# yangdongchao/Text-to-sound-Synthesis

Hardware: NVIDIA H100
Metric: clips/sec (10s audio, 100 diffusion steps) (higher is better)
Workload: dtype f16x3

## Files before the change

### include/diffsound_b200.h

```cpp
#ifndef DIFFSOUND_B200_H
#define DIFFSOUND_B200_H

#include <stdint.h>

#ifdef __cplusplus
extern "C" {
#endif

#define DSB_VERSION 100

#define DSB_DTYPE_TF32 0
#define DSB_DTYPE_BF16 1
#define DSB_DTYPE_F16 2

#define DSB_GEMM_GELU2 1
#define DSB_GEMM_ROUND_TF32 2
#define DSB_GEMM_OUT_BF16 4
#define DSB_GEMM_LRELU 8
#define DSB_GEMM_TANH 16
#define DSB_GEMM_OUT_F16 256
#define DSB_GEMM_RES_BEFORE_ACT 128
#define DSB_GEMM_DUAL_LRELU 4096
#define DSB_GEMM_NO_STORE 16384
#define DSB_GEMM_RELU 32768
// ... 33 lines not shown
  int b_mn_major;
  int use_tap_wcol;
  int tap_wcol[32];
  long long w_cols;
  long long split_off;
  long long dual_off;
  int out_col_group;
  int out_col_group_stride;
  const void* A2;
  long long a2_rows, a2_cols, lda2, a2_batch_stride;
  int tap_a2[32];
  float* amax_out;
  int resident_w;
  int schedule;
} dsb_gemm_desc;
int dsb_gemm_ex(const dsb_gemm_desc* desc, void* stream);

int dsb_gemm_f32(const float* A, const float* W, const float* bias, const float* residual, float* out, int M, int N, int K,
                 long long lda, long long ldw, long long ldo, long long ld_res, int flags, void* stream);

int dsb_round_tf32(const float* in, float* out, long long n, void* stream);
int dsb_f32_to_bf16(const float* in, void* out_bf16, long long n, void* stream);
int dsb_f32_to_f16(const float* in, void* out_f16, long long n, void* stream);
int dsb_split_f16(const float* in, long long ld_in, void* out_f16, long long ld_out, long long lo_off, long long rows, int C, float scale,
                  void* stream);
int dsb_split_tf32(const float* in, long long ld_in, float* out, long long ld_out, long long rows, int C, int Cp, int w_format, void* stream);

int dsb_embed_tokens(const int64_t* ids, const float* emb, const float* height_emb, const float* width_emb, float* out, int B, int L,
                     int D, int H, int W, int num_embed, int* err_flag, void* stream);

int dsb_layernorm(const float* x, void* out, const float* gamma, const float* beta, int rows, int D, float eps, int flags, void* stream);

int dsb_ada_layernorm(const float* x, void* out, const float* table, const int64_t* t, int B, int L, int D, int T, float eps, int flags,
                      void* stream);

int dsb_l2_normalize_rows(float* x, long long rows, int D, void* stream);

int dsb_silu(const float* in, float* out, long long n, void* stream);

int dsb_attention(const float* q, long long ldq, const float* k, long long ldk, const float* v, long long ldv, float* o, long long ldo,
                  int B, int H, int Lq, int Lk, float scale, int flags, void* stream);

#define DSB_ATTN_CAUSAL 1024
int dsb_attention_f16(const void* q, long long ldq, const void* k, long long ldk, const void* v, long long ldv, void* o, long long ldo,
                      int B, int H, int Lq, int Lk, float scale, int flags, void* stream);

int dsb_attention_tc(const void* q, long long ldq, const void* k, long long ldk, const void* v, long long ldv, void* o, long long ldo,
                     int B, int H, int Lq, int Lk, float scale, void* stream);
int dsb_attention_tc2(const void* q, long long ldq, const void* k, long long ldk, const void* v, long long ldv, void* o, long long ldo,
                      int B, int H, int Lq, int Lk, float scale, void* stream);
int dsb_attention_tc_split(const void* q, long long ldq, long long q_lo_off, const void* k, long long ldk, long long k_lo_off, const void* v,
                           long long ldv, long long v_lo_off, void* o, long long ldo, long long o_lo_off, int B, int H, int Lq, int Lk,
                           float scale, void* stream);


#define DSB_STAGE_INPUT_LOGPROB 1
#define DSB_STAGE_SKIP_POSTERIOR 2
#define DSB_STAGE_SKIP_SAMPLE 4
int dsb_posterior_sample(const float* logits, const int64_t* x_t, const int64_t* t, const int64_t* t_post, const float* uniform,
                         const float* sched, int64_t* x_next, float* log_prob_out, int B, int K, int L, int T, int trunc_mode,
                         float trunc_r, int trunc_k, int stage_flags, void* stream);

int dsb_posterior_sample_loop(const float* logits, int64_t* x, int64_t* t, int64_t* t_post, const float* sched, unsigned long long* ctrl,
                              const int64_t* t_sched, const int64_t* t_post_sched, int B, int K, int L, int T, int trunc_mode, float trunc_r,
                              int trunc_k, void* stream);
int dsb_posterior_sample_wide(const float* logits, const int64_t* x_t, const int64_t* t, const int64_t* t_post, const float* uniform,
                              const float* sched, int64_t* x_next, float* log_prob_out, int B, int K, int L, int T, int trunc_mode,
                              float trunc_r, int trunc_k, int stage_flags, void* stream);
int dsb_posterior_sample_wide_loop(const float* logits, int64_t* x, int64_t* t, int64_t* t_post, const float* sched, unsigned long long* ctrl,
                                   const int64_t* t_sched, const int64_t* t_post_sched, int B, int K, int L, int T, int trunc_mode, float trunc_r,
                                   int trunc_k, void* stream);
int dsb_aten_uniform(float* out, long long n, unsigned long long seed, unsigned long long offset, unsigned long long nthreads, void* stream);
int dsb_aten_exponential(float* out, long long n, unsigned long long seed, unsigned long long offset, unsigned long long nthreads, void* stream);

int dsb_ar_embed(const float* cond, const float* tok_emb, const float* pos_emb, const int64_t* ids, long long ids_ld, float* x,
                 const unsigned long long* ctrl, int B, int Tc, int V, int D, int* err_flag, void* stream);
int dsb_ar_attention(const float* qkv, long long ld_qkv, float* k_cache, float* v_cache, long long cache_ld, int max_pos, void* out, long long ld_out,
                     long long lo_off, const unsigned long long* ctrl, int B, int H, int head_dim, float scale, void* stream);
int dsb_gelu_erf_split(const float* in, long long ld_in, void* out, long long ld_out, long long lo_off, int rows, int C, void* stream);
int dsb_ar_sample(const float* logits, long long ld_logits, int64_t* ids, long long ids_ld, unsigned long long* ctrl, int B, int V, int Tc,
                  float temperature, int top_k, int do_sample, float* probs_out, float* logits_hist, long long hist_ld, int* err_flag, void* stream);

int dsb_codebook_gather_padded(const int64_t* ids, const float* codebook, float* out, int B, int H, int W, int E, int n_codes, int flags,
                               int* err_flag, void* stream);
int dsb_groupnorm_stats(const float* x, double* stats, int B, int P, int C, int groups, void* stream);
int dsb_groupnorm_apply(const float* x, const double* stats, const float* gamma, const float* beta, float* out, int B, int H, int W, int C,
                        int groups, float eps, int flags, int Lp, void* stream);
int dsb_upsample2x_padded(const float* in, float* out, int B, int H, int W, int C, int flags, void* stream);
int dsb_softmax_rows(float* x, long long rows, int n_valid, int ld, int flags, void* stream);
int dsb_space_to_depth_padded(const float* in, float* out, int B, int H, int W, int C, int flags, void* stream);
int dsb_row_argmin(const float* x, long long ld, long long rows, int n, int64_t* out, void* stream);
int dsb_tokens_add_to_padded(const float* tok, float* xpad, int B, int H, int W, int C, int Lp, void* stream);

int dsb_lrelu_pad(const float* in, float* out, int B, int T, int C, int pad, float slope, int reflect, int in_channel_major, int flags,
                  void* stream);
int dsb_mel_pack_f16(const float* mel, void* out_f16, int B, int Cm, int T, int pad, int Kp, void* stream);
int dsb_edge_pad_f16(void* state_f16, long long ld, long long batch_stride, int B, int T, int P, int d, int col0, int ncols, int reflect,
                     void* stream);
int dsb_conv_out_pair(const void* state, long long ld, long long batch_stride, int B, int T, int row0, int col0, int cs, int kt, const float* w,
                      const float* bias, float scale, float* out, void* stream);


int dsb_mel_stem(const float* x, const float* mean, const float* stdv, const float* w, const float* bias, float scale, void* out, int B, int F, int T,
                 int Cout, int Hp, int Wp, int y0, int x0, void* stream);
int dsb_pair_space_to_depth(const void* in, int Hpi, int Wpi, int y0, int x0, int H, int W, void* out, int Hpo, int Wpo, int oy0, int ox0, int B, int C,
                            void* stream);
// ... 43 lines not shown
```

### text-to-sound-synthesis_b200/_lib.py

```python
from __future__ import annotations

import ctypes as C
import os

_HERE = os.path.dirname(os.path.abspath(__file__))
LIB_PATH = os.path.join(_HERE, "libdiffsound_b200.so")

c_vp, c_i, c_ll, c_f = C.c_void_p, C.c_int, C.c_longlong, C.c_float


class GemmDesc(C.Structure):
    _fields_ = [
        ("A", c_vp), ("W", c_vp), ("bias", c_vp), ("residual", c_vp), ("out", c_vp),
        ("M", c_i), ("N", c_i), ("K", c_i), ("batch", c_i),
        ("a_rows", c_ll), ("lda", c_ll), ("ldw", c_ll), ("ldo", c_ll), ("ld_res", c_ll),
        ("a_batch_stride", c_ll), ("w_batch_stride", c_ll), ("out_batch_stride", c_ll), ("res_batch_stride", c_ll),
        ("dtype", c_i), ("flags", c_i), ("num_taps", c_i), ("tap_shift", c_i * 32), ("tap_acol", c_i * 32), ("a_cols", c_ll),
        ("geo_P", c_i), ("geo_Wp", c_i), ("geo_y0", c_i), ("geo_y1", c_i), ("geo_x0", c_i), ("geo_x1", c_i),
        ("alpha", c_f), ("block_n", c_i), ("max_ctas", c_i), ("cta_pair", c_i), ("a_mn_major", c_i), ("b_mn_major", c_i),
        ("use_tap_wcol", c_i), ("tap_wcol", c_i * 32), ("w_cols", c_ll), ("split_off", c_ll),
        ("dual_off", c_ll), ("out_col_group", c_i), ("out_col_group_stride", c_i), ("A2", c_vp),
        ("a2_rows", c_ll), ("a2_cols", c_ll), ("lda2", c_ll), ("a2_batch_stride", c_ll), ("tap_a2", c_i * 32), ("amax_out", c_vp), ("resident_w", c_i),
        ("schedule", c_i),
    ]


SIGNATURES = {
    "dsb_version": [],
    "dsb_device_info": [C.POINTER(c_i)] * 3,
    "dsb_gemm_ex": [C.POINTER(GemmDesc), c_vp],
    "dsb_gemm_f32": [c_vp] * 5 + [c_i] * 3 + [c_ll] * 4 + [c_i, c_vp],
    "dsb_round_tf32": [c_vp, c_vp, c_ll, c_vp],
    "dsb_f32_to_bf16": [c_vp, c_vp, c_ll, c_vp],
    "dsb_f32_to_f16": [c_vp, c_vp, c_ll, c_vp],
    "dsb_silu": [c_vp, c_vp, c_ll, c_vp],
    "dsb_split_f16": [c_vp, c_ll, c_vp, c_ll, c_ll, c_ll, c_i, c_f, c_vp],
    "dsb_attention_tc_split": [c_vp, c_ll, c_ll, c_vp, c_ll, c_ll, c_vp, c_ll, c_ll, c_vp, c_ll, c_ll, c_i, c_i, c_i, c_i, c_f, c_vp],
    "dsb_l2_normalize_rows": [c_vp, c_ll, c_i, c_vp],
    "dsb_split_tf32": [c_vp, c_ll, c_vp, c_ll, c_ll, c_i, c_i, c_i, c_vp],
    "dsb_embed_tokens": [c_vp] * 5 + [c_i] * 6 + [c_vp, c_vp],
    "dsb_layernorm": [c_vp] * 4 + [c_i, c_i, c_f, c_i, c_vp],
    "dsb_ada_layernorm": [c_vp] * 4 + [c_i] * 4 + [c_f, c_i, c_vp],
    "dsb_attention": [c_vp, c_ll, c_vp, c_ll, c_vp, c_ll, c_vp, c_ll, c_i, c_i, c_i, c_i, c_f, c_i, c_vp],
    "dsb_codebook_gather_padded": [c_vp] * 3 + [c_i] * 6 + [c_vp, c_vp],
    "dsb_groupnorm_stats": [c_vp, c_vp] + [c_i] * 4 + [c_vp],
    "dsb_groupnorm_apply": [c_vp] * 5 + [c_i] * 5 + [c_f, c_i, c_i, c_vp],
    "dsb_upsample2x_padded": [c_vp, c_vp] + [c_i] * 5 + [c_vp],
    "dsb_softmax_rows": [c_vp, c_ll, c_i, c_i, c_i, c_vp],
    "dsb_space_to_depth_padded": [c_vp, c_vp] + [c_i] * 5 + [c_vp],
    "dsb_row_argmin": [c_vp, c_ll, c_ll, c_i, c_vp, c_vp],
    "dsb_tokens_add_to_padded": [c_vp, c_vp] + [c_i] * 5 + [c_vp],
    "dsb_lrelu_pad": [c_vp, c_vp] + [c_i] * 4 + [c_f, c_i, c_i, c_i, c_vp],
    "dsb_mel_pack_f16": [c_vp, c_vp] + [c_i] * 5 + [c_vp],
    "dsb_edge_pad_f16": [c_vp, c_ll, c_ll] + [c_i] * 7 + [c_vp],
    "dsb_conv_out_pair": [c_vp, c_ll, c_ll] + [c_i] * 6 + [c_vp, c_vp, c_f, c_vp, c_vp],
    "dsb_attention_f16": [c_vp, c_ll, c_vp, c_ll, c_vp, c_ll, c_vp, c_ll, c_i, c_i, c_i, c_i, c_f, c_i, c_vp],
    "dsb_attention_tc2": [c_vp, c_ll, c_vp, c_ll, c_vp, c_ll, c_vp, c_ll, c_i, c_i, c_i, c_i, c_f, c_vp],
    "dsb_attention_tc": [c_vp, c_ll, c_vp, c_ll, c_vp, c_ll, c_vp, c_ll, c_i, c_i, c_i, c_i, c_f, c_vp],
    "dsb_posterior_sample": [c_vp] * 8 + [c_i] * 5 + [c_f, c_i, c_i, c_vp],
    "dsb_posterior_sample_loop": [c_vp] * 8 + [c_i] * 5 + [c_f, c_i, c_vp],
    "dsb_posterior_sample_wide": [c_vp] * 8 + [c_i] * 5 + [c_f, c_i, c_i, c_vp],
    "dsb_posterior_sample_wide_loop": [c_vp] * 8 + [c_i] * 5 + [c_f, c_i, c_vp],
    "dsb_aten_uniform": [c_vp, c_ll, C.c_ulonglong, C.c_ulonglong, C.c_ulonglong, c_vp],
    "dsb_aten_exponential": [c_vp, c_ll, C.c_ulonglong, C.c_ulonglong, C.c_ulonglong, c_vp],
    "dsb_ar_embed": [c_vp] * 4 + [c_ll, c_vp, c_vp] + [c_i] * 4 + [c_vp, c_vp],
    "dsb_ar_attention": [c_vp, c_ll, c_vp, c_vp, c_ll, c_i, c_vp, c_ll, c_ll, c_vp, c_i, c_i, c_i, c_f, c_vp],
    "dsb_gelu_erf_split": [c_vp, c_ll, c_vp, c_ll, c_ll, c_i, c_i, c_vp],
    "dsb_ar_sample": [c_vp, c_ll, c_vp, c_ll, c_vp, c_i, c_i, c_i, c_f, c_i, c_i, c_vp, c_vp, c_ll, c_vp, c_vp],
    "dsb_mel_stem": [c_vp] * 5 + [c_f, c_vp] + [c_i] * 8 + [c_vp],
    "dsb_pair_space_to_depth": [c_vp] + [c_i] * 6 + [c_vp] + [c_i] * 6 + [c_vp],
    "dsb_pair_maxpool3s2": [c_vp] + [c_i] * 6 + [c_vp, c_ll, c_ll] + [c_i] * 6 + [c_f, c_vp],
    "dsb_pair_avgpool3": [c_vp] + [c_i] * 6 + [c_vp, c_ll, c_ll, c_i, c_i, c_vp],
    "dsb_pair_channel_mean": [c_vp, c_ll, c_ll] + [c_i] * 8 + [c_f, c_vp, c_vp],
    "dsb_q_sample": [c_vp] * 5 + [c_i] * 4 + [c_vp],
    "dsb_train_loss": [c_vp] * 16 + [c_i] * 4 + [c_f, c_i, c_f, c_f, c_i, c_vp],
    "dsb_transpose": [c_vp, c_ll, c_ll, c_vp, c_ll, c_ll, c_i, c_i, c_i, c_i, c_vp],
    "dsb_heads_split": [c_vp, c_ll, c_vp, c_i, c_i, c_i, c_i, c_vp],
    "dsb_heads_merge": [c_vp, c_vp, c_ll, c_i, c_i, c_i, c_i, c_vp],
    "dsb_cast_scale": [c_vp, c_vp, c_ll, c_vp, c_i, c_vp],
    "dsb_colsum": [c_vp, c_ll, c_vp, c_ll, c_i, c_i, c_vp],
    "dsb_gelu2_fwd": [c_vp, c_vp, c_ll, c_i, c_vp],
    "dsb_gelu2_bwd": [c_vp, c_vp, c_vp, c_ll, c_i, c_vp],
    "dsb_silu_bwd": [c_vp, c_vp, c_vp, c_ll, c_vp],
    "dsb_gather_rows": [c_vp, c_vp, c_vp, c_i, c_i, c_vp],
    "dsb_scatter_add_rows": [c_vp, c_vp, c_vp, c_i, c_i, c_vp],
    "dsb_layernorm_bwd": [c_vp] * 6 + [c_ll, c_i, c_f, c_vp, c_i, c_vp],
    "dsb_ada_layernorm_bwd": [c_vp] * 6 + [c_i, c_i, c_i, c_f, c_vp, c_i, c_vp],
    "dsb_softmax_fwd": [c_vp, c_ll, c_vp, c_ll, c_ll, c_i, c_i, c_vp],
    "dsb_softmax_bwd": [c_vp, c_ll, c_vp, c_ll, c_vp, c_ll, c_ll, c_i, c_f, c_i, c_vp],
    "dsb_embed_bwd": [c_vp] * 5 + [c_i] * 6 + [c_vp],
# ... 28 lines not shown
```

### text-to-sound-synthesis_b200/csrc/wgmma.cuh

```cuda
#pragma once
#include "common.cuh"
#include "diffsound_b200.h"

namespace dsb {

template <int KIND, int TA, int TB>
__device__ __forceinline__ void wgmma_m64n128(float (&d)[64], uint64_t da, uint64_t db, uint32_t scale_d) {
  static_assert(KIND != DSB_DTYPE_TF32 || (TA == 0 && TB == 0), "tf32 wgmma takes K-major operands only");
  if constexpr (KIND == DSB_DTYPE_TF32) {
    asm volatile(
        "{\n\t.reg .pred p;\n\tsetp.ne.b32 p, %66, 0;\n\t"
        "wgmma.mma_async.sync.aligned.m64n128k8.f32.tf32.tf32 "
        "{%0, %1, %2, %3, %4, %5, %6, %7, %8, %9, %10, %11, %12, %13, %14, %15, %16, %17, %18, %19, %20, %21, %22, %23, %24, %25, %26, %27, %28, %29, %30, %31, %32, %33, %34, %35, %36, %37, %38, %39, %40, %41, %42, %43, %44, %45, %46, %47, %48, %49, %50, %51, %52, %53, %54, %55, %56, %57, %58, %59, %60, %61, %62, %63}, "
        "%64, %65, p, 1, 1;\n\t}"
        : "+f"(d[0]), "+f"(d[1]), "+f"(d[2]), "+f"(d[3]), "+f"(d[4]), "+f"(d[5]), "+f"(d[6]), "+f"(d[7]), "+f"(d[8]), "+f"(d[9]), "+f"(d[10]), "+f"(d[11]), "+f"(d[12]), "+f"(d[13]), "+f"(d[14]), "+f"(d[15]), "+f"(d[16]), "+f"(d[17]), "+f"(d[18]), "+f"(d[19]), "+f"(d[20]), "+f"(d[21]), "+f"(d[22]), "+f"(d[23]), "+f"(d[24]), "+f"(d[25]), "+f"(d[26]), "+f"(d[27]), "+f"(d[28]), "+f"(d[29]), "+f"(d[30]), "+f"(d[31]), "+f"(d[32]), "+f"(d[33]), "+f"(d[34]), "+f"(d[35]), "+f"(d[36]), "+f"(d[37]), "+f"(d[38]), "+f"(d[39]), "+f"(d[40]), "+f"(d[41]), "+f"(d[42]), "+f"(d[43]), "+f"(d[44]), "+f"(d[45]), "+f"(d[46]), "+f"(d[47]), "+f"(d[48]), "+f"(d[49]), "+f"(d[50]), "+f"(d[51]), "+f"(d[52]), "+f"(d[53]), "+f"(d[54]), "+f"(d[55]), "+f"(d[56]), "+f"(d[57]), "+f"(d[58]), "+f"(d[59]), "+f"(d[60]), "+f"(d[61]), "+f"(d[62]), "+f"(d[63])
        : "l"(da), "l"(db), "r"(scale_d));
  } else if constexpr (KIND == DSB_DTYPE_BF16) {
    asm volatile(
        "{\n\t.reg .pred p;\n\tsetp.ne.b32 p, %66, 0;\n\t"
        "wgmma.mma_async.sync.aligned.m64n128k16.f32.bf16.bf16 "
        "{%0, %1, %2, %3, %4, %5, %6, %7, %8, %9, %10, %11, %12, %13, %14, %15, %16, %17, %18, %19, %20, %21, %22, %23, %24, %25, %26, %27, %28, %29, %30, %31, %32, %33, %34, %35, %36, %37, %38, %39, %40, %41, %42, %43, %44, %45, %46, %47, %48, %49, %50, %51, %52, %53, %54, %55, %56, %57, %58, %59, %60, %61, %62, %63}, "
        "%64, %65, p, 1, 1, %67, %68;\n\t}"
        : "+f"(d[0]), "+f"(d[1]), "+f"(d[2]), "+f"(d[3]), "+f"(d[4]), "+f"(d[5]), "+f"(d[6]), "+f"(d[7]), "+f"(d[8]), "+f"(d[9]), "+f"(d[10]), "+f"(d[11]), "+f"(d[12]), "+f"(d[13]), "+f"(d[14]), "+f"(d[15]), "+f"(d[16]), "+f"(d[17]), "+f"(d[18]), "+f"(d[19]), "+f"(d[20]), "+f"(d[21]), "+f"(d[22]), "+f"(d[23]), "+f"(d[24]), "+f"(d[25]), "+f"(d[26]), "+f"(d[27]), "+f"(d[28]), "+f"(d[29]), "+f"(d[30]), "+f"(d[31]), "+f"(d[32]), "+f"(d[33]), "+f"(d[34]), "+f"(d[35]), "+f"(d[36]), "+f"(d[37]), "+f"(d[38]), "+f"(d[39]), "+f"(d[40]), "+f"(d[41]), "+f"(d[42]), "+f"(d[43]), "+f"(d[44]), "+f"(d[45]), "+f"(d[46]), "+f"(d[47]), "+f"(d[48]), "+f"(d[49]), "+f"(d[50]), "+f"(d[51]), "+f"(d[52]), "+f"(d[53]), "+f"(d[54]), "+f"(d[55]), "+f"(d[56]), "+f"(d[57]), "+f"(d[58]), "+f"(d[59]), "+f"(d[60]), "+f"(d[61]), "+f"(d[62]), "+f"(d[63])
        : "l"(da), "l"(db), "r"(scale_d), "n"(TA), "n"(TB));
  } else {
    asm volatile(
        "{\n\t.reg .pred p;\n\tsetp.ne.b32 p, %66, 0;\n\t"
        "wgmma.mma_async.sync.aligned.m64n128k16.f32.f16.f16 "
        "{%0, %1, %2, %3, %4, %5, %6, %7, %8, %9, %10, %11, %12, %13, %14, %15, %16, %17, %18, %19, %20, %21, %22, %23, %24, %25, %26, %27, %28, %29, %30, %31, %32, %33, %34, %35, %36, %37, %38, %39, %40, %41, %42, %43, %44, %45, %46, %47, %48, %49, %50, %51, %52, %53, %54, %55, %56, %57, %58, %59, %60, %61, %62, %63}, "
        "%64, %65, p, 1, 1, %67, %68;\n\t}"
        : "+f"(d[0]), "+f"(d[1]), "+f"(d[2]), "+f"(d[3]), "+f"(d[4]), "+f"(d[5]), "+f"(d[6]), "+f"(d[7]), "+f"(d[8]), "+f"(d[9]), "+f"(d[10]), "+f"(d[11]), "+f"(d[12]), "+f"(d[13]), "+f"(d[14]), "+f"(d[15]), "+f"(d[16]), "+f"(d[17]), "+f"(d[18]), "+f"(d[19]), "+f"(d[20]), "+f"(d[21]), "+f"(d[22]), "+f"(d[23]), "+f"(d[24]), "+f"(d[25]), "+f"(d[26]), "+f"(d[27]), "+f"(d[28]), "+f"(d[29]), "+f"(d[30]), "+f"(d[31]), "+f"(d[32]), "+f"(d[33]), "+f"(d[34]), "+f"(d[35]), "+f"(d[36]), "+f"(d[37]), "+f"(d[38]), "+f"(d[39]), "+f"(d[40]), "+f"(d[41]), "+f"(d[42]), "+f"(d[43]), "+f"(d[44]), "+f"(d[45]), "+f"(d[46]), "+f"(d[47]), "+f"(d[48]), "+f"(d[49]), "+f"(d[50]), "+f"(d[51]), "+f"(d[52]), "+f"(d[53]), "+f"(d[54]), "+f"(d[55]), "+f"(d[56]), "+f"(d[57]), "+f"(d[58]), "+f"(d[59]), "+f"(d[60]), "+f"(d[61]), "+f"(d[62]), "+f"(d[63])
        : "l"(da), "l"(db), "r"(scale_d), "n"(TA), "n"(TB));
  }
}

template <int TA, int TB>
__device__ __forceinline__ void wgmma_m64n64_f16_ss(float (&d)[32], uint64_t da, uint64_t db, uint32_t scale_d) {
  asm volatile(
      "{\n\t.reg .pred p;\n\tsetp.ne.b32 p, %34, 0;\n\t"
      "wgmma.mma_async.sync.aligned.m64n64k16.f32.f16.f16 "
      "{%0, %1, %2, %3, %4, %5, %6, %7, %8, %9, %10, %11, %12, %13, %14, %15, %16, %17, %18, %19, %20, %21, %22, %23, %24, %25, %26, %27, %28, %29, %30, %31}, "
      "%32, %33, p, 1, 1, %35, %36;\n\t}"
      : "+f"(d[0]), "+f"(d[1]), "+f"(d[2]), "+f"(d[3]), "+f"(d[4]), "+f"(d[5]), "+f"(d[6]), "+f"(d[7]), "+f"(d[8]), "+f"(d[9]), "+f"(d[10]), "+f"(d[11]), "+f"(d[12]), "+f"(d[13]), "+f"(d[14]), "+f"(d[15]), "+f"(d[16]), "+f"(d[17]), "+f"(d[18]), "+f"(d[19]), "+f"(d[20]), "+f"(d[21]), "+f"(d[22]), "+f"(d[23]), "+f"(d[24]), "+f"(d[25]), "+f"(d[26]), "+f"(d[27]), "+f"(d[28]), "+f"(d[29]), "+f"(d[30]), "+f"(d[31])
      : "l"(da), "l"(db), "r"(scale_d), "n"(TA), "n"(TB));
}

template <int TB>
__device__ __forceinline__ void wgmma_m64n64_f16_rs(float (&d)[32], const uint32_t (&a)[4], uint64_t db, uint32_t scale_d) {
  asm volatile(
      "{\n\t.reg .pred p;\n\tsetp.ne.b32 p, %37, 0;\n\t"
      "wgmma.mma_async.sync.aligned.m64n64k16.f32.f16.f16 "
      "{%0, %1, %2, %3, %4, %5, %6, %7, %8, %9, %10, %11, %12, %13, %14, %15, %16, %17, %18, %19, %20, %21, %22, %23, %24, %25, %26, %27, %28, %29, %30, %31}, "
      "{%32, %33, %34, %35}, %36, p, 1, 1, %38;\n\t}"
      : "+f"(d[0]), "+f"(d[1]), "+f"(d[2]), "+f"(d[3]), "+f"(d[4]), "+f"(d[5]), "+f"(d[6]), "+f"(d[7]), "+f"(d[8]), "+f"(d[9]), "+f"(d[10]), "+f"(d[11]), "+f"(d[12]), "+f"(d[13]), "+f"(d[14]), "+f"(d[15]), "+f"(d[16]), "+f"(d[17]), "+f"(d[18]), "+f"(d[19]), "+f"(d[20]), "+f"(d[21]), "+f"(d[22]), "+f"(d[23]), "+f"(d[24]), "+f"(d[25]), "+f"(d[26]), "+f"(d[27]), "+f"(d[28]), "+f"(d[29]), "+f"(d[30]), "+f"(d[31])
      : "r"(a[0]), "r"(a[1]), "r"(a[2]), "r"(a[3]), "l"(db), "r"(scale_d), "n"(TB));
}

}
```

### text-to-sound-synthesis_b200/engine.py

```python
from __future__ import annotations

import math
import copy
from typing import Dict, Optional

import torch

from . import ops


class DenoiserEngine:
    def __init__(self, transformer, precision: str = "f16x3"):
        if precision not in ("f16x3", "f16", "tf32", "fp32"):
            raise ValueError("precision must be 'f16x3', 'f16', 'tf32' or 'fp32'")
        self.m = transformer
        self.precision = precision
        self.packed = False
        self._ws: Dict[int, dict] = {}
        self.launches_per_forward = 0
        self.generation = 0
        self._param_sig = None

    def __deepcopy__(self, memo):
        return DenoiserEngine(memo.get(id(self.m), self.m), precision=self.precision)
# ... 115 lines not shown
    @torch.no_grad()
    def forward(self, ids: torch.Tensor, kv_all: torch.Tensor, t: torch.Tensor, Lc: int, out: Optional[torch.Tensor] = None) -> torch.Tensor:
        if not self.packed:
            self.repack()
        B, L = ids.shape
        D, H = self.D, self.H
        ws = self.workspace(B, L)
        x, h, qkv, att, q2, hid = ws["x"], ws["h"], ws["qkv"], ws["att"], ws["q2"], ws["hid"]
        rnd = self.precision == "tf32"
        if self.precision == "f16x3":
            return self._forward_split(ids, kv_all, t, Lc, out)
        x2 = x.view(B * L, D)
        h2 = h.view(B * L, D)
        scale = 1.0 / math.sqrt(64)
        n = 0
        ops.embed_tokens(ids, self.emb, self.hemb, self.wemb, out=x, err_flag=ws["err"]); n += 1
        for li, lay in enumerate(self.layers):
            ops.ada_layernorm(x, lay["tab1"], t, out=h, round_out=rnd)
            self._linear(h2, lay["wqkv"], lay["bqkv"], out=qkv)
            if self.precision == "f16" and L <= 272:
                ops.attention_tc(qkv[:, :D], qkv[:, D:2 * D], qkv[:, 2 * D:], att, B=B, H=H, Lq=L, Lk=L, scale=scale)
            else:
                ops.attention(qkv[:, :D], qkv[:, D:2 * D], qkv[:, 2 * D:], att, B=B, H=H, Lq=L, Lk=L, scale=scale, round_out=rnd)
            self._linear(att, lay["wo1"], lay["bo1"], residual=x2, out=x2)
            ops.ada_layernorm(x, lay["tab2"], t, out=h, round_out=rnd)
            self._linear(h2, lay["wq2"], lay["bq2"], out=q2)
            kv = kv_all[:, li * 2 * D:(li + 1) * 2 * D]
            if self.precision == "f16" and Lc <= 272:
                ops.attention_tc(q2, kv[:, :D], kv[:, D:], att, B=B, H=H, Lq=L, Lk=Lc, scale=scale)
            else:
                ops.attention(q2, kv[:, :D], kv[:, D:], att, B=B, H=H, Lq=L, Lk=Lc, scale=scale, round_out=rnd)
            self._linear(att, lay["wo2"], lay["bo2"], residual=x2, out=x2)
            ops.layernorm(x, lay["g2"], lay["b2"], out=h, eps=lay["eps2"], round_out=rnd)
            self._linear(h2, lay["w1"], lay["b1"], out=hid, gelu=True, round_out=rnd)
            self._linear(hid, lay["w2"], lay["bm2"], residual=x2, out=x2)
            n += 11
        ops.layernorm(x, self.gf, self.bf, out=h, eps=self.epsf, round_out=rnd)
        logits = ws["logits"] if out is None else out
        self._linear(h2, self.wlog, self.blog, out=logits.view(B * L, self.K))
        self.launches_per_forward = n + 2
        return logits

    @torch.no_grad()
    def _forward_split(self, ids, kv_all, t, Lc, out=None):
        B, L = ids.shape
        D, H = self.D, self.H
        ws = self.workspace(B, L)
        x, h, qkv, att, q2, hid = ws["x"], ws["h"], ws["qkv"], ws["att"], ws["q2"], ws["hid"]
        M = B * L
        x2, h2 = x.view(M, D), h.view(M, 2 * D)
        scale = 1.0 / math.sqrt(64)
        kv_lo = self.n_layer * 2 * D
        n = 0
        ops.embed_tokens(ids, self.emb, self.hemb, self.wemb, out=x, err_flag=ws["err"]); n += 1
        for li, lay in enumerate(self.layers):
            ops.ada_layernorm(x, lay["tab1"], t, out=h, split=True)
            self._linear(h2, lay["wqkv"], lay["bqkv"], out=qkv, split_out=True)
            ops.attention_tc_split(qkv[:, :D], qkv[:, D:2 * D], qkv[:, 2 * D:3 * D], att[:, :D], q_lo=3 * D, k_lo=3 * D, v_lo=3 * D, o_lo=D,
                                   B=B, H=H, Lq=L, Lk=L, scale=scale)
            self._linear(att, lay["wo1"], lay["bo1"], residual=x2, out=x2)
            ops.ada_layernorm(x, lay["tab2"], t, out=h, split=True)
            self._linear(h2, lay["wq2"], lay["bq2"], out=q2, split_out=True)
            kv = kv_all[:, li * 2 * D:]
            ops.attention_tc_split(q2[:, :D], kv[:, :D], kv[:, D:2 * D], att[:, :D], q_lo=D, k_lo=kv_lo, v_lo=kv_lo, o_lo=D,
                                   B=B, H=H, Lq=L, Lk=Lc, scale=scale)
            self._linear(att, lay["wo2"], lay["bo2"], residual=x2, out=x2)
            ops.layernorm(x, lay["g2"], lay["b2"], out=h, eps=lay["eps2"], split=True)
            self._linear(h2, lay["w1"], lay["b1"], out=hid, gelu=True, split_out=True)
            self._linear(hid, lay["w2"], lay["bm2"], residual=x2, out=x2)
            n += 11
        ops.layernorm(x, self.gf, self.bf, out=h, eps=self.epsf, split=True)
        logits = ws["logits"] if out is None else out
        self._linear(h2, self.wlog, self.blog, out=logits.view(M, self.K))
        self.launches_per_forward = n + 2
        return logits


class _SplitWeight:
    __slots__ = ("pair", "alpha")

    def __init__(self, pair, alpha):
        self.pair, self.alpha = pair, alpha

    @property
    def shape(self):
        return (self.pair.shape[0], self.pair.shape[1] // 2)
```

### text-to-sound-synthesis_b200/ops.py

```python
from __future__ import annotations

import ctypes as C
from typing import Optional, Sequence

import torch

from . import _lib

TF32, BF16, F16 = 0, 1, 2
GELU2, ROUND_TF32, OUT_BF16, LRELU, TANH, GN_SWISH, GN_COMPACT, RES_BEFORE_ACT, OUT_F16, SPLIT_OUT = 1, 2, 4, 8, 16, 32, 64, 128, 256, 512
OUT_F16_SPLIT = 2048
DUAL_LRELU = 4096
SPLIT_OUT_F16 = 8192
NO_STORE = 16384
RELU = 32768


def _stream() -> int:
    return torch.cuda.current_stream().cuda_stream


def _ptr(t: Optional[torch.Tensor]):
    return None if t is None else t.data_ptr()

# ... 274 lines not shown


def l2_normalize_rows_(x):
    _need_cuda(x)
    D = x.shape[-1]
    _lib.check(_lib.lib().dsb_l2_normalize_rows(x.data_ptr(), x.numel() // D, D, _stream()), "dsb_l2_normalize_rows")
    return x


ATTN_CAUSAL = 1024


def attention(q, k, v, out, *, B, H, Lq, Lk, scale, round_out=False, causal=False):
    _need_cuda(q, k, v, out)
    for t_ in (q, k, v, out):
        if t_.stride(-1) != 1:
            raise RuntimeError("attention operands must be contiguous in the head dimension")
    if q.dtype == torch.float16:
        if k.dtype != torch.float16 or v.dtype != torch.float16:
            raise RuntimeError("attention: q, k, v must share a dtype")
        _lib.check(_lib.lib().dsb_attention_f16(q.data_ptr(), q.stride(0), k.data_ptr(), k.stride(0), v.data_ptr(), v.stride(0), out.data_ptr(),
                                                out.stride(0), B, H, Lq, Lk, scale, _out_flags(out, False) | (ATTN_CAUSAL if causal else 0), _stream()),
                   "dsb_attention_f16")
        return out
    if causal:
        raise RuntimeError("causal attention is implemented for fp16 operands")
    _lib.check(_lib.lib().dsb_attention(q.data_ptr(), q.stride(0), k.data_ptr(), k.stride(0), v.data_ptr(), v.stride(0), out.data_ptr(), out.stride(0),
                                        B, H, Lq, Lk, scale, _out_flags(out, round_out), _stream()), "dsb_attention")
    return out


STAGE_INPUT_LOGPROB, STAGE_SKIP_POSTERIOR, STAGE_SKIP_SAMPLE = 1, 2, 4


def attention_tc(q, k, v, out, *, B, H, Lq, Lk, scale, pipelined=True):
    _need_cuda(q, k, v, out)
    if not all(t_.dtype == torch.float16 and t_.stride(-1) == 1 for t_ in (q, k, v, out)):
        raise RuntimeError("attention_tc needs fp16 tensors contiguous in the head dimension")
    fn = _lib.lib().dsb_attention_tc2 if pipelined else _lib.lib().dsb_attention_tc
    _lib.check(fn(q.data_ptr(), q.stride(0), k.data_ptr(), k.stride(0), v.data_ptr(), v.stride(0), out.data_ptr(), out.stride(0),
                  B, H, Lq, Lk, scale, _stream()), "dsb_attention_tc")
    return out


def attention_tc_split(q, k, v, out, *, q_lo, k_lo, v_lo, o_lo, B, H, Lq, Lk, scale):
    _need_cuda(q, k, v, out)
    if not all(t_.dtype == torch.float16 and t_.stride(-1) == 1 for t_ in (q, k, v, out)):
        raise RuntimeError("attention_tc_split needs fp16 tensors contiguous in the head dimension")
    _lib.check(_lib.lib().dsb_attention_tc_split(q.data_ptr(), q.stride(0), q_lo, k.data_ptr(), k.stride(0), k_lo, v.data_ptr(), v.stride(0), v_lo,
                                                 out.data_ptr(), out.stride(0), o_lo, B, H, Lq, Lk, scale, _stream()), "dsb_attention_tc_split")
    return out


def posterior_sample(inp, x_t, t, uniform, sched, *, T, trunc_mode=1, trunc_r=0.85, trunc_k=0, t_post=None, x_next=None, log_prob_out=None,
                     stage=0):
    return _posterior_sample("dsb_posterior_sample", inp, x_t, t, uniform, sched, T, trunc_mode, trunc_r, trunc_k, t_post, x_next, log_prob_out, stage)


def posterior_sample_wide(inp, x_t, t, uniform, sched, *, T, trunc_mode=1, trunc_r=0.85, trunc_k=0, t_post=None, x_next=None, log_prob_out=None,
                          stage=0):
    return _posterior_sample("dsb_posterior_sample_wide", inp, x_t, t, uniform, sched, T, trunc_mode, trunc_r, trunc_k, t_post, x_next, log_prob_out,
                             stage)


WARP_SAMPLER_MAX_K = 1055
WIDE_SAMPLER_MAX_K = 4095


def _posterior_sample(fn, inp, x_t, t, uniform, sched, T, trunc_mode, trunc_r, trunc_k, t_post, x_next, log_prob_out, stage):
    _need_cuda(inp, x_t, t, uniform, sched, log_prob_out)
    if stage & STAGE_INPUT_LOGPROB:
        B, C_, L = inp.shape
        K = C_ - 1
    else:
        B, L, K = inp.shape
    for t_ in (inp, x_t, uniform, sched, log_prob_out, t, t_post):
        if t_ is not None and not t_.is_contiguous():
            raise RuntimeError("posterior_sample needs contiguous tensors")
    if uniform is not None and tuple(uniform.shape) != (B, K + 1, L):
        raise RuntimeError(f"uniform must be (B,K+1,L)={(B, K + 1, L)}, got {tuple(uniform.shape)}")
    if sched is not None and tuple(sched.shape) != (8, T + 1):
        raise RuntimeError("sched must be (8, T+1)")
    if not (stage & STAGE_SKIP_SAMPLE) and x_next is None:
        x_next = torch.empty((B, L), dtype=torch.int64, device=inp.device)
    _lib.check(getattr(_lib.lib(), fn)(inp.data_ptr(), _ptr(x_t), _ptr(t), _ptr(t_post), _ptr(uniform), _ptr(sched), _ptr(x_next),
                                       _ptr(log_prob_out), B, K, L, T, trunc_mode, trunc_r, trunc_k, stage, _stream()), fn)
    return x_next


def aten_rand_geometry(numel: int, device=None):
    pr = torch.cuda.get_device_properties(device if device is not None else torch.cuda.current_device())
    grid = min(pr.multi_processor_count * (pr.max_threads_per_multi_processor // 256), (numel + 255) // 256)
    return 256 * grid, ((numel - 1) // (256 * grid * 4) + 1) * 4


def aten_uniform(numel: int, seed: int, offset: int, device=None) -> torch.Tensor:
    out = torch.empty(numel, dtype=torch.float32, device=device if device is not None else "cuda")
    nthreads, _ = aten_rand_geometry(numel, out.device)
    _lib.check(_lib.lib().dsb_aten_uniform(out.data_ptr(), numel, seed & (2 ** 64 - 1), offset, nthreads, _stream()), "dsb_aten_uniform")
    return out


def posterior_sample_loop(logits, x, t, t_post, sched, ctrl, t_sched, t_post_sched, *, T, trunc_mode=1, trunc_r=0.85, trunc_k=0):
    return _posterior_sample_loop("dsb_posterior_sample_loop", logits, x, t, t_post, sched, ctrl, t_sched, t_post_sched, T, trunc_mode, trunc_r, trunc_k)


# ... 211 lines not shown
```

Measured before the change: 8.866.

## Add persistent attention kernel keeping per-head K/V resident in shared memory

```diff
diff --git a/include/diffsound_b200.h b/include/diffsound_b200.h
--- a/include/diffsound_b200.h
+++ b/include/diffsound_b200.h
@@ -109,6 +109,9 @@
 int dsb_attention_tc_split(const void* q, long long ldq, long long q_lo_off, const void* k, long long ldk, long long k_lo_off, const void* v,
                            long long ldv, long long v_lo_off, void* o, long long ldo, long long o_lo_off, int B, int H, int Lq, int Lk,
                            float scale, void* stream);
+int dsb_attention_split_resident(const void* q, long long ldq, long long q_lo_off, const void* k, long long ldk, long long k_lo_off, const void* v,
+                                 long long ldv, long long v_lo_off, void* o, long long ldo, long long o_lo_off, int B, int H, int Lq, int Lk,
+                                 float scale, void* stream);
 
 
 #define DSB_STAGE_INPUT_LOGPROB 1
diff --git a/text-to-sound-synthesis_b200/_lib.py b/text-to-sound-synthesis_b200/_lib.py
--- a/text-to-sound-synthesis_b200/_lib.py
+++ b/text-to-sound-synthesis_b200/_lib.py
@@ -36,6 +36,7 @@
     "dsb_silu": [c_vp, c_vp, c_ll, c_vp],
     "dsb_split_f16": [c_vp, c_ll, c_vp, c_ll, c_ll, c_ll, c_i, c_f, c_vp],
     "dsb_attention_tc_split": [c_vp, c_ll, c_ll, c_vp, c_ll, c_ll, c_vp, c_ll, c_ll, c_vp, c_ll, c_ll, c_i, c_i, c_i, c_i, c_f, c_vp],
+    "dsb_attention_split_resident": [c_vp, c_ll, c_ll, c_vp, c_ll, c_ll, c_vp, c_ll, c_ll, c_vp, c_ll, c_ll, c_i, c_i, c_i, c_i, c_f, c_vp],
     "dsb_l2_normalize_rows": [c_vp, c_ll, c_i, c_vp],
     "dsb_split_tf32": [c_vp, c_ll, c_vp, c_ll, c_ll, c_i, c_i, c_i, c_vp],
     "dsb_embed_tokens": [c_vp] * 5 + [c_i] * 6 + [c_vp, c_vp],
diff --git a/text-to-sound-synthesis_b200/csrc/attention_split_resident.cu b/text-to-sound-synthesis_b200/csrc/attention_split_resident.cu
--- /dev/null
+++ b/text-to-sound-synthesis_b200/csrc/attention_split_resident.cu
@@ -0,0 +1,305 @@
+#include "common.cuh"
+#include "diffsound_b200.h"
+#include "wgmma.cuh"
+#include <cuda_fp16.h>
+
+namespace dsb {
+namespace {
+constexpr int AR_HD = 64;
+constexpr int AR_TILE = 64 * 128;
+constexpr int AR_MAX_CHUNKS = 5;
+constexpr int AR_CHUNK_BYTES = 4 * AR_TILE;
+constexpr int AR_Q_BYTES = 2 * AR_TILE;
+constexpr int AR_THREADS = 384;
+constexpr int AR_SMEM = AR_MAX_CHUNKS * AR_CHUNK_BYTES + 4 * AR_Q_BYTES + (2 * AR_MAX_CHUNKS + 8) * 8 + 1024;
+static_assert(AR_SMEM <= 227 * 1024, "resident K / V + 4 Q slots must fit one SM's shared memory");
+
+struct ArParams {
+  int H, Lq, Lk;
+  int n_chunks, n_tiles, n_heads;
+  int last_w;
+  int q_lo_col, k_lo_col, v_lo_col;
+  long long ldo, o_lo_off;
+  __half* o;
+  float scale_log2e;
+};
+
+__device__ __forceinline__ float ar_ex2(float x) {
+  float y;
+  asm("ex2.approx.ftz.f32 %0, %1;" : "=f"(y) : "f"(x));
+  return y;
+}
+__device__ __forceinline__ void ar_pack_pair(float a, float b, uint32_t& hi, uint32_t& lo) {
+  const __half2 h = __floats2half2_rn(a, b);
+  const __half2 l = __floats2half2_rn(a - __low2float(h), b - __high2float(h));
+  hi = *reinterpret_cast<const uint32_t*>(&h);
+  lo = *reinterpret_cast<const uint32_t*>(&l);
+}
+__device__ __forceinline__ void ldmatrix_x4(uint32_t (&r)[4], uint32_t addr) {
+  asm volatile("ldmatrix.sync.aligned.m8n8.x4.shared.b16 {%0, %1, %2, %3}, [%4];" : "=r"(r[0]), "=r"(r[1]), "=r"(r[2]), "=r"(r[3]) : "r"(addr));
+}
+
+struct ArTile {
+  uint32_t qh[4][4], ql[4][4];
+  float o[32];
+  float m0, m1, l0, l1;
+};
+
+template <int W>
+__device__ __forceinline__ void ar_chunk(const ArParams& p, ArTile& T, const uint8_t* stage, uint64_t* full, uint64_t* empty, int c, uint32_t par,
+                                         bool release, int lane) {
+  const int t = lane & 3;
+  mbar_wait(&full[c], par);
+  const uint32_t sk = smem_u32(stage);
+  float s[W / 2], part[32];
+  wgmma_fence_regs(s);
+  wgmma_fence();
+#pragma unroll
+  for (int k = 0; k < 4; ++k) {
+    const uint64_t dkh = make_sw128_kmajor_desc(sk) + 2 * k, dkl = make_sw128_kmajor_desc(sk + AR_TILE) + 2 * k;
+    wgmma_m64nN_f16_rs<W, 0>(s, T.ql[k], dkh, k != 0 ? 1u : 0u);
+    wgmma_m64nN_f16_rs<W, 0>(s, T.qh[k], dkl, 1u);
+    wgmma_m64nN_f16_rs<W, 0>(s, T.qh[k], dkh, 1u);
+  }
+  wgmma_commit();
+  wgmma_wait<0>();
+  wgmma_fence_regs(s);
+
+  if ((c + 1) * 64 > p.Lk) {
+#pragma unroll
+    for (int j = 0; j < W / 8; ++j) {
+      const int key = c * 64 + j * 8 + 2 * t;
+      if (key >= p.Lk) { s[4 * j] = -INFINITY; s[4 * j + 2] = -INFINITY; }
+      if (key + 1 >= p.Lk) { s[4 * j + 1] = -INFINITY; s[4 * j + 3] = -INFINITY; }
+    }
+  }
+  float mx0 = -INFINITY, mx1 = -INFINITY;
+#pragma unroll
+  for (int j = 0; j < W / 8; ++j) {
+    mx0 = fmaxf(mx0, fmaxf(s[4 * j], s[4 * j + 1]));
+    mx1 = fmaxf(mx1, fmaxf(s[4 * j + 2], s[4 * j + 3]));
+  }
+  mx0 = fmaxf(mx0, __shfl_xor_sync(0xffffffffu, mx0, 1)); mx0 = fmaxf(mx0, __shfl_xor_sync(0xffffffffu, mx0, 2));
+  mx1 = fmaxf(mx1, __shfl_xor_sync(0xffffffffu, mx1, 1)); mx1 = fmaxf(mx1, __shfl_xor_sync(0xffffffffu, mx1, 2));
+  const float mn0 = fmaxf(T.m0, mx0), mn1 = fmaxf(T.m1, mx1);
+  const float c0 = ar_ex2((T.m0 - mn0) * p.scale_log2e), c1 = ar_ex2((T.m1 - mn1) * p.scale_log2e);
+  const float ms0 = mn0 * p.scale_log2e, ms1 = mn1 * p.scale_log2e;
+  T.m0 = mn0; T.m1 = mn1;
+  T.l0 *= c0; T.l1 *= c1;
+#pragma unroll
+  for (int j = 0; j < 8; ++j) { T.o[4 * j] *= c0; T.o[4 * j + 1] *= c0; T.o[4 * j + 2] *= c1; T.o[4 * j + 3] *= c1; }
+#pragma unroll
+  for (int j = 0; j < W / 8; ++j) {
+    s[4 * j] = ar_ex2(fmaf(s[4 * j], p.scale_log2e, -ms0)); s[4 * j + 1] = ar_ex2(fmaf(s[4 * j + 1], p.scale_log2e, -ms0));
+    s[4 * j + 2] = ar_ex2(fmaf(s[4 * j + 2], p.scale_log2e, -ms1)); s[4 * j + 3] = ar_ex2(fmaf(s[4 * j + 3], p.scale_log2e, -ms1));
+    T.l0 += s[4 * j] + s[4 * j + 1];
+    T.l1 += s[4 * j + 2] + s[4 * j + 3];
+  }
+  uint32_t ph[W / 16][4], pl[W / 16][4];
+#pragma unroll
+  for (int kk = 0; kk < W / 16; ++kk) {
+    ar_pack_pair(s[8 * kk], s[8 * kk + 1], ph[kk][0], pl[kk][0]);
+    ar_pack_pair(s[8 * kk + 2], s[8 * kk + 3], ph[kk][1], pl[kk][1]);
+    ar_pack_pair(s[8 * kk + 4], s[8 * kk + 5], ph[kk][2], pl[kk][2]);
+    ar_pack_pair(s[8 * kk + 6], s[8 * kk + 7], ph[kk][3], pl[kk][3]);
+  }
+  wgmma_fence_regs(part);
+  wgmma_fence();
+#pragma unroll
+  for (int kk = 0; kk < W / 16; ++kk) {
+    const uint64_t dvh = make_sw128_desc(sk + 2 * AR_TILE, AR_TILE) + 128 * kk, dvl = make_sw128_desc(sk + 3 * AR_TILE, AR_TILE) + 128 * kk;
+    wgmma_m64n64_f16_rs<1>(part, pl[kk], dvh, kk != 0 ? 1u : 0u);
+    wgmma_m64n64_f16_rs<1>(part, ph[kk], dvl, 1u);
+    wgmma_m64n64_f16_rs<1>(part, ph[kk], dvh, 1u);
+  }
+  wgmma_commit();
+  wgmma_wait<0>();
+  wgmma_fence_regs(part);
+  if (release && lane == 0) mbar_arrive(&empty[c]);
+#pragma unroll
+  for (int i = 0; i < 32; ++i) T.o[i] += part[i];
+}
+
+__device__ __forceinline__ void ar_tile(const ArParams& p, const uint8_t* kv, uint64_t* full, uint64_t* empty, uint32_t par, bool release, uint8_t* sq,
+                                        int b, int h, int tile, int wg, int wq, int lane) {
+  const int t = lane & 3;
+  ArTile T;
+  {
+    const int r = wq * 16 + (lane & 7) + ((lane >> 3) & 1) * 8;
+    const uint32_t row = smem_u32(sq) + r * 128;
+#pragma unroll
+    for (int k = 0; k < 4; ++k) {
+      const uint32_t a = row + (((2 * k + (lane >> 4)) ^ (r & 7)) << 4);
+      ldmatrix_x4(T.qh[k], a);
+      ldmatrix_x4(T.ql[k], a + AR_TILE);
+    }
+  }
+#pragma unroll
+  for (int i = 0; i < 32; ++i) T.o[i] = 0.f;
+  T.m0 = -INFINITY; T.m1 = -INFINITY; T.l0 = 0.f; T.l1 = 0.f;
+  for (int c = 0; c < p.n_chunks - 1; ++c) ar_chunk<64>(p, T, kv + c * AR_CHUNK_BYTES, full, empty, c, par, release, lane);
+  const int c = p.n_chunks - 1;
+  switch (p.last_w) {
+    case 16: ar_chunk<16>(p, T, kv + c * AR_CHUNK_BYTES, full, empty, c, par, release, lane); break;
+    case 32: ar_chunk<32>(p, T, kv + c * AR_CHUNK_BYTES, full, empty, c, par, release, lane); break;
+    case 48: ar_chunk<48>(p, T, kv + c * AR_CHUNK_BYTES, full, empty, c, par, release, lane); break;
+    default: ar_chunk<64>(p, T, kv + c * AR_CHUNK_BYTES, full, empty, c, par, release, lane); break;
+  }
+
+  float l0 = T.l0, l1 = T.l1;
+  l0 += __shfl_xor_sync(0xffffffffu, l0, 1); l0 += __shfl_xor_sync(0xffffffffu, l0, 2);
+  l1 += __shfl_xor_sync(0xffffffffu, l1, 1); l1 += __shfl_xor_sync(0xffffffffu, l1, 2);
+  const float i0 = __fdividef(1.0f, l0), i1 = __fdividef(1.0f, l1);
+  named_bar_sync(1 + wg, 128);
+  const int r0 = wq * 16 + (lane >> 2), r1 = r0 + 8;
+#pragma unroll
+  for (int j = 0; j < 8; ++j) {
+    uint32_t hi, lo;
+    ar_pack_pair(T.o[4 * j] * i0, T.o[4 * j + 1] * i0, hi, lo);
+    *reinterpret_cast<uint32_t*>(sq + r0 * 128 + ((j ^ (r0 & 7)) << 4) + 4 * t) = hi;
+    *reinterpret_cast<uint32_t*>(sq + AR_TILE + r0 * 128 + ((j ^ (r0 & 7)) << 4) + 4 * t) = lo;
+    ar_pack_pair(T.o[4 * j + 2] * i1, T.o[4 * j + 3] * i1, hi, lo);
+    *reinterpret_cast<uint32_t*>(sq + r1 * 128 + ((j ^ (r1 & 7)) << 4) + 4 * t) = hi;
+    *reinterpret_cast<uint32_t*>(sq + AR_TILE + r1 * 128 + ((j ^ (r1 & 7)) << 4) + 4 * t) = lo;
+  }
+  named_bar_sync(1 + wg, 128);
+  const int ct = wq * 32 + lane;
+  __half* ob = p.o + (long long)b * p.Lq * p.ldo + h * AR_HD;
+#pragma unroll
+  for (int i = 0; i < 8; ++i) {
+    const int idx = ct + 128 * i, half = idx >> 9, r = (idx >> 3) & 63, ch = idx & 7;
+    const int row = tile * 64 + r;
+    if (row < p.Lq)
+      *reinterpret_cast<uint4*>(ob + (long long)row * p.ldo + half * p.o_lo_off + ch * 8) =
+          *reinterpret_cast<const uint4*>(sq + half * AR_TILE + r * 128 + ((ch ^ (r & 7)) << 4));
+  }
+  fence_proxy_async_smem();
+}
+
+__global__ void __launch_bounds__(AR_THREADS, 1)
+attention_split_resident_kernel(const __grid_constant__ CUtensorMap map_q, const __grid_constant__ CUtensorMap map_k,
+                                const __grid_constant__ CUtensorMap map_v, const __grid_constant__ ArParams p) {
+  extern __shared__ uint8_t smem_raw[];
+  uint8_t* smem = reinterpret_cast<uint8_t*>((reinterpret_cast<uintptr_t>(smem_raw) + 1023) & ~uintptr_t(1023));
+  uint8_t* kv = smem;
+  uint8_t* qbuf = kv + AR_MAX_CHUNKS * AR_CHUNK_BYTES;
+  uint64_t* full = reinterpret_cast<uint64_t*>(qbuf + 4 * AR_Q_BYTES);
+  uint64_t* empty = full + AR_MAX_CHUNKS;
+  uint64_t* q_full = empty + AR_MAX_CHUNKS;
+  uint64_t* q_empty = q_full + 4;
+  const int warp = threadIdx.x >> 5, lane = threadIdx.x & 31;
+
+  if (threadIdx.x == 0) {
+    for (int s = 0; s < AR_MAX_CHUNKS; ++s) {
+      mbar_init(&full[s], 1);
+      mbar_init(&empty[s], 8);
+    }
+    for (int i = 0; i < 4; ++i) {
+      mbar_init(&q_full[i], 1);
+      mbar_init(&q_empty[i], 4);
+    }
+    fence_barrier_init();
+    prefetch_tmap(&map_q); prefetch_tmap(&map_k); prefetch_tmap(&map_v);
+  }
+  __syncthreads();
+  pdl_wait();
+  pdl_trigger();
+
+  if (warp < 4) {
+    setmaxnreg_dec<40>();
+    if (threadIdx.x == 0) {
+      int qn0 = 0, qn1 = 0;
+      for (int i = 0, bh = blockIdx.x; bh < p.n_heads; ++i, bh += gridDim.x) {
+        const int b = bh / p.H, h = bh - b * p.H;
+        auto load_q = [&](int tile) {
+          const int w = (i + tile) & 1;
+          const int qn = w ? qn1 : qn0;
+          const int q = 2 * w + (qn & 1);
+          mbar_wait(&q_empty[q], ((qn >> 1) & 1) ^ 1);
+          mbar_arrive_expect_tx(&q_full[q], AR_Q_BYTES);
+          uint8_t* dst = qbuf + q * AR_Q_BYTES;
+          tma_load_3d(&map_q, &q_full[q], dst, h * AR_HD, tile * 64, b);
+          tma_load_3d(&map_q, &q_full[q], dst + AR_TILE, p.q_lo_col + h * AR_HD, tile * 64, b);
+          if (w) ++qn1; else ++qn0;
+        };
+        load_q(0);
+        if (p.n_tiles > 1) load_q(1);
+        for (int c = 0; c < p.n_chunks; ++c) {
+          mbar_wait(&empty[c], (i & 1) ^ 1);
+          mbar_arrive_expect_tx(&full[c], AR_CHUNK_BYTES);
+          uint8_t* st = kv + c * AR_CHUNK_BYTES;
+          tma_load_3d(&map_k, &full[c], st, h * AR_HD, c * 64, b);
+          tma_load_3d(&map_k, &full[c], st + AR_TILE, p.k_lo_col + h * AR_HD, c * 64, b);
+          tma_load_3d(&map_v, &full[c], st + 2 * AR_TILE, h * AR_HD, c * 64, b);
+          tma_load_3d(&map_v, &full[c], st + 3 * AR_TILE, p.v_lo_col + h * AR_HD, c * 64, b);
+        }
+        for (int tile = 2; tile < p.n_tiles; ++tile) load_q(tile);
+      }
+    }
+  } else {
+    setmaxnreg_inc<232>();
+    const int wg = (warp >> 2) - 1, wq = warp & 3;
+    int qn = 0;
+    for (int i = 0, bh = blockIdx.x; bh < p.n_heads; ++i, bh += gridDim.x) {
+      const int b = bh / p.H, h = bh - b * p.H;
+      const uint32_t par = i & 1;
+      const int first = (i + wg) & 1;
+      if (first >= p.n_tiles) {
+        for (int c = 0; c < p.n_chunks; ++c) {
+          mbar_wait(&full[c], par);
+          if (lane == 0) mbar_arrive(&empty[c]);
+        }
+        continue;
+      }
+      for (int tile = first; tile < p.n_tiles; tile += 2) {
+        const int q = 2 * wg + (qn & 1);
+        mbar_wait(&q_full[q], (qn >> 1) & 1);
+        ar_tile(p, kv, full, empty, par, tile + 2 >= p.n_tiles, qbuf + q * AR_Q_BYTES, b, h, tile, wg, wq, lane);
+        __syncwarp();
+        if (lane == 0) mbar_arrive(&q_empty[q]);
+        ++qn;
+      }
+    }
+  }
+}
+}
+}
+
+extern "C" int dsb_attention_split_resident(const void* q, long long ldq, long long q_lo_off, const void* k, long long ldk, long long k_lo_off,
+                                            const void* v, long long ldv, long long v_lo_off, void* o, long long ldo, long long o_lo_off, int B, int H,
+                                            int Lq, int Lk, float scale, void* stream) {
+  using namespace dsb;
+  DSB_REQUIRE(B > 0 && H > 0 && Lq > 0 && Lk > 0, "dsb_attention_split_resident: need B, H, Lq, Lk > 0");
+  DSB_REQUIRE(Lk <= AR_MAX_CHUNKS * 64, "dsb_attention_split_resident: Lk = %d > %d keys do not fit in shared memory; use dsb_attention_tc_split", Lk,
+              AR_MAX_CHUNKS * 64);
+  DSB_REQUIRE(ldo % 8 == 0 && o_lo_off % 8 == 0 && (reinterpret_cast<uintptr_t>(o) & 15) == 0,
+              "dsb_attention_split_resident: o must be 16-byte aligned, ldo / o_lo_off %% 8 == 0");
+  DSB_REQUIRE(q_lo_off >= (long long)H * AR_HD && k_lo_off >= (long long)H * AR_HD && v_lo_off >= (long long)H * AR_HD && o_lo_off >= (long long)H * AR_HD,
+              "dsb_attention_split_resident: the lo halves must not overlap the hi halves");
+  DSB_REQUIRE(q_lo_off + (long long)H * AR_HD <= ldq && k_lo_off + (long long)H * AR_HD <= ldk && v_lo_off + (long long)H * AR_HD <= ldv,
+              "dsb_attention_split_resident: lo halves must lie inside a row (lo_off + H*64 <= ld)");
+  DSB_REQUIRE(ldq % 8 == 0 && (reinterpret_cast<uintptr_t>(q) & 15) == 0, "dsb_attention_split_resident: q must be 16-byte aligned, ldq %% 8 == 0 (TMA)");
+  const long long heads = (long long)B * H;
+  DSB_REQUIRE(heads < (1LL << 31), "dsb_attention_split_resident: too many (batch, head) units");
+  ArParams p{};
+  p.H = H; p.Lq = Lq; p.Lk = Lk;
+  p.n_chunks = (Lk + 63) / 64;
+  p.n_tiles = (Lq + 63) / 64;
+  p.n_heads = (int)heads;
+  p.last_w = ((Lk - 64 * (p.n_chunks - 1)) + 15) & ~15;
+  p.q_lo_col = (int)q_lo_off; p.k_lo_col = (int)k_lo_off; p.v_lo_col = (int)v_lo_off;
+  p.ldo = ldo; p.o_lo_off = o_lo_off; p.o = (__half*)o;
+  p.scale_log2e = scale * 1.4426950408889634f;
+  CUtensorMap mq, mk, mv;
+  if (make_operand_map(&mq, q, DSB_DTYPE_F16, q_lo_off + (long long)H * AR_HD, Lq, B, ldq, (long long)Lq * ldq, 64)) return 3;
+  if (make_operand_map(&mk, k, DSB_DTYPE_F16, k_lo_off + (long long)H * AR_HD, Lk, B, ldk, (long long)Lk * ldk, 64)) return 3;
+  if (make_operand_map(&mv, v, DSB_DTYPE_F16, v_lo_off + (long long)H * AR_HD, Lk, B, ldv, (long long)Lk * ldv, 64)) return 3;
+  static bool attr_set = false;
+  if (!attr_set) {
+    DSB_CHECK_CUDA(cudaFuncSetAttribute(attention_split_resident_kernel, cudaFuncAttributeMaxDynamicSharedMemorySize, AR_SMEM));
+    attr_set = true;
+  }
+  const int grid = min(p.n_heads, sm_count());
+  DSB_CHECK_CUDA(launch_pdl(attention_split_resident_kernel, dim3(grid), dim3(AR_THREADS), AR_SMEM, (cudaStream_t)stream, mq, mk, mv, p));
+  return 0;
+}
diff --git a/text-to-sound-synthesis_b200/csrc/wgmma.cuh b/text-to-sound-synthesis_b200/csrc/wgmma.cuh
--- a/text-to-sound-synthesis_b200/csrc/wgmma.cuh
+++ b/text-to-sound-synthesis_b200/csrc/wgmma.cuh
@@ -56,4 +56,36 @@
       : "r"(a[0]), "r"(a[1]), "r"(a[2]), "r"(a[3]), "l"(db), "r"(scale_d), "n"(TB));
 }
 
+template <int N, int TB>
+__device__ __forceinline__ void wgmma_m64nN_f16_rs(float (&d)[N / 2], const uint32_t (&a)[4], uint64_t db, uint32_t scale_d) {
+  static_assert(N == 16 || N == 32 || N == 48 || N == 64, "m64nNk16: N = 16, 32, 48 or 64");
+  if constexpr (N == 64) {
+    wgmma_m64n64_f16_rs<TB>(d, a, db, scale_d);
+  } else if constexpr (N == 48) {
+    asm volatile(
+        "{\n\t.reg .pred p;\n\tsetp.ne.b32 p, %29, 0;\n\t"
+        "wgmma.mma_async.sync.aligned.m64n48k16.f32.f16.f16 "
+        "{%0, %1, %2, %3, %4, %5, %6, %7, %8, %9, %10, %11, %12, %13, %14, %15, %16, %17, %18, %19, %20, %21, %22, %23}, "
+        "{%24, %25, %26, %27}, %28, p, 1, 1, %30;\n\t}"
+        : "+f"(d[0]), "+f"(d[1]), "+f"(d[2]), "+f"(d[3]), "+f"(d[4]), "+f"(d[5]), "+f"(d[6]), "+f"(d[7]), "+f"(d[8]), "+f"(d[9]), "+f"(d[10]), "+f"(d[11]), "+f"(d[12]), "+f"(d[13]), "+f"(d[14]), "+f"(d[15]), "+f"(d[16]), "+f"(d[17]), "+f"(d[18]), "+f"(d[19]), "+f"(d[20]), "+f"(d[21]), "+f"(d[22]), "+f"(d[23])
+        : "r"(a[0]), "r"(a[1]), "r"(a[2]), "r"(a[3]), "l"(db), "r"(scale_d), "n"(TB));
+  } else if constexpr (N == 32) {
+    asm volatile(
+        "{\n\t.reg .pred p;\n\tsetp.ne.b32 p, %21, 0;\n\t"
+        "wgmma.mma_async.sync.aligned.m64n32k16.f32.f16.f16 "
+        "{%0, %1, %2, %3, %4, %5, %6, %7, %8, %9, %10, %11, %12, %13, %14, %15}, "
+        "{%16, %17, %18, %19}, %20, p, 1, 1, %22;\n\t}"
+        : "+f"(d[0]), "+f"(d[1]), "+f"(d[2]), "+f"(d[3]), "+f"(d[4]), "+f"(d[5]), "+f"(d[6]), "+f"(d[7]), "+f"(d[8]), "+f"(d[9]), "+f"(d[10]), "+f"(d[11]), "+f"(d[12]), "+f"(d[13]), "+f"(d[14]), "+f"(d[15])
+        : "r"(a[0]), "r"(a[1]), "r"(a[2]), "r"(a[3]), "l"(db), "r"(scale_d), "n"(TB));
+  } else {
+    asm volatile(
+        "{\n\t.reg .pred p;\n\tsetp.ne.b32 p, %13, 0;\n\t"
+        "wgmma.mma_async.sync.aligned.m64n16k16.f32.f16.f16 "
+        "{%0, %1, %2, %3, %4, %5, %6, %7}, "
+        "{%8, %9, %10, %11}, %12, p, 1, 1, %14;\n\t}"
+        : "+f"(d[0]), "+f"(d[1]), "+f"(d[2]), "+f"(d[3]), "+f"(d[4]), "+f"(d[5]), "+f"(d[6]), "+f"(d[7])
+        : "r"(a[0]), "r"(a[1]), "r"(a[2]), "r"(a[3]), "l"(db), "r"(scale_d), "n"(TB));
+  }
 }
+
+}
diff --git a/text-to-sound-synthesis_b200/engine.py b/text-to-sound-synthesis_b200/engine.py
--- a/text-to-sound-synthesis_b200/engine.py
+++ b/text-to-sound-synthesis_b200/engine.py
@@ -191,18 +191,21 @@
         scale = 1.0 / math.sqrt(64)
         kv_lo = self.n_layer * 2 * D
         n = 0
+
+        def attn(lk):
+            return ops.attention_split_resident if lk <= 320 else ops.attention_tc_split
         ops.embed_tokens(ids, self.emb, self.hemb, self.wemb, out=x, err_flag=ws["err"]); n += 1
         for li, lay in enumerate(self.layers):
             ops.ada_layernorm(x, lay["tab1"], t, out=h, split=True)
             self._linear(h2, lay["wqkv"], lay["bqkv"], out=qkv, split_out=True)
-            ops.attention_tc_split(qkv[:, :D], qkv[:, D:2 * D], qkv[:, 2 * D:3 * D], att[:, :D], q_lo=3 * D, k_lo=3 * D, v_lo=3 * D, o_lo=D,
-                                   B=B, H=H, Lq=L, Lk=L, scale=scale)
+            attn(L)(qkv[:, :D], qkv[:, D:2 * D], qkv[:, 2 * D:3 * D], att[:, :D], q_lo=3 * D, k_lo=3 * D, v_lo=3 * D, o_lo=D,
+                    B=B, H=H, Lq=L, Lk=L, scale=scale)
             self._linear(att, lay["wo1"], lay["bo1"], residual=x2, out=x2)
             ops.ada_layernorm(x, lay["tab2"], t, out=h, split=True)
             self._linear(h2, lay["wq2"], lay["bq2"], out=q2, split_out=True)
             kv = kv_all[:, li * 2 * D:]
-            ops.attention_tc_split(q2[:, :D], kv[:, :D], kv[:, D:2 * D], att[:, :D], q_lo=D, k_lo=kv_lo, v_lo=kv_lo, o_lo=D,
-                                   B=B, H=H, Lq=L, Lk=Lc, scale=scale)
+            attn(Lc)(q2[:, :D], kv[:, :D], kv[:, D:2 * D], att[:, :D], q_lo=D, k_lo=kv_lo, v_lo=kv_lo, o_lo=D,
+                     B=B, H=H, Lq=L, Lk=Lc, scale=scale)
             self._linear(att, lay["wo2"], lay["bo2"], residual=x2, out=x2)
             ops.layernorm(x, lay["g2"], lay["b2"], out=h, eps=lay["eps2"], split=True)
             self._linear(h2, lay["w1"], lay["b1"], out=hid, gelu=True, split_out=True)
diff --git a/text-to-sound-synthesis_b200/ops.py b/text-to-sound-synthesis_b200/ops.py
--- a/text-to-sound-synthesis_b200/ops.py
+++ b/text-to-sound-synthesis_b200/ops.py
@@ -350,6 +350,16 @@
     return out
 
 
+def attention_split_resident(q, k, v, out, *, q_lo, k_lo, v_lo, o_lo, B, H, Lq, Lk, scale):
+    _need_cuda(q, k, v, out)
+    if not all(t_.dtype == torch.float16 and t_.stride(-1) == 1 for t_ in (q, k, v, out)):
+        raise RuntimeError("attention_split_resident needs fp16 tensors contiguous in the head dimension")
+    _lib.check(_lib.lib().dsb_attention_split_resident(q.data_ptr(), q.stride(0), q_lo, k.data_ptr(), k.stride(0), k_lo, v.data_ptr(), v.stride(0),
+                                                       v_lo, out.data_ptr(), out.stride(0), o_lo, B, H, Lq, Lk, scale, _stream()),
+               "dsb_attention_split_resident")
+    return out
+
+
 def posterior_sample(inp, x_t, t, uniform, sched, *, T, trunc_mode=1, trunc_r=0.85, trunc_k=0, t_post=None, x_next=None, log_prob_out=None,
                      stage=0):
     return _posterior_sample("dsb_posterior_sample", inp, x_t, t, uniform, sched, T, trunc_mode, trunc_r, trunc_k, t_post, x_next, log_prob_out, stage)
```

Result: faster. 8.981 (median of 6 runs) (+1.3%).
